# sandialabs/calibr8

Measured on AMD Instinct MI355X. Metric: element Jacobian assemblies/sec, 1M hex8 J2-plasticity fp64, higher is better.
Workload: dtype f64

## Files before the change

### calibr8_amd/csrc/c8_assemble_node.hpp

```cpp
#pragma once

#include "c8_assemble_wave.hpp"

#ifdef C8_STAMPS
#define C8_NSTAMP(i) ex.stamp_node(ga.stamps, node, i)
#else
#define C8_NSTAMP(i)
#endif

namespace c8 {

template <class M, class = void> struct has_closed_form_rows : std::false_type {};
template <class M> struct has_closed_form_rows<M, std::enable_if_t<M::HAS_CLOSED_FORM_ROWS>> : std::true_type {};

template <class E, class ModelD, int MAXDEG, bool MANY> struct NodeShared {
  static constexpr int NR = ModelD::NROW;
  static constexpr int LDR = NR + 4;
  static_assert(LDR % 2 == 0 && (E::NP0 * LDR * 8) % 256 == 128, "record stride: 16-byte aligned, element groups 32 banks apart");
  static constexpr int NREC = 8 * E::NP0 * LDR, NACC = MAXDEG * 16;
  alignas(16) double buf[MANY ? NREC + NACC : (NREC > NACC ? NREC : NACC)];
  alignas(16) double nodal[8][E::NN][4];
  double nshape[8];
  double el[8][2];
  double bsum[4];
  C8_HD double* rec(int s, int pt) { return buf + (s * E::NP0 + pt) * LDR; }
  C8_HD double* img() { return buf + (MANY ? NREC : 0); }
  C8_HD static int img01(int deg) { return 9 * deg; }
  C8_HD static int img10(int deg) { return 12 * deg; }
  C8_HD static int img11(int deg) { return 15 * deg; }
};

C8_HD double const* at_byte(double const* p, int off) { return reinterpret_cast<double const*>(reinterpret_cast<char const*>(p) + off); }

#ifndef C8_TUNE_NODE_HAHEAD
#define C8_TUNE_NODE_HAHEAD 3
#endif

template <int MAXDEG> struct NodeLane {
  static constexpr int N00 = (9 * MAXDEG + 63) / 64, N01 = (3 * MAXDEG + 63) / 64;
  double J[16];
  double a00[N00], a01[N01], a10[N01], a11;
  double bold;
  double rs;
  int e, a, pos;
  bool valid;
};

C8_HD constexpr int hex_code(int n) { return n ^ ((n >> 1) & 1); }
template <class E> C8_HD void hex_pattern(int j, double* v) {
  double c[3], w;
  E::point(0, 7, c, w);
  double const a = 1. + ((j & 1) ? c[0] : -c[0]), b = 1. + ((j & 2) ? c[1] : -c[1]), d = 1. + ((j & 4) ? c[2] : -c[2]);
  v[0] = 0.125 * a * b * d;
  v[1] = 0.125 * b * d;
  v[2] = 0.125 * a * d;
  v[3] = 0.125 * a * b;
}

template <class E> struct HexShape {
  double c[3];
  C8_HD static HexShape of_point(int pt) {
    double w;
    HexShape h;
    E::point(0, pt, h.c, w);
    return h;
  }
  C8_HD double at_node(int n) const {
    double const sx = ((n ^ (n >> 1)) & 1) ? 1. : -1., sy = ((n >> 1) & 1) ? 1. : -1., sz = ((n >> 2) & 1) ? 1. : -1.;
    return 0.125 * (1. + sx * c[0]) * (1. + sy * c[1]) * (1. + sz * c[2]);
  }
  C8_HD static HexShape of_node(int n) {
    HexShape h;
    E::sign(n, h.c[0], h.c[1], h.c[2]);
    return h;
  }
  C8_HD double at_point(int pt) const {
    double xi[3], w;
    E::point(0, pt, xi, w);
    return 0.125 * (1. + c[0] * xi[0]) * (1. + c[1] * xi[1]) * (1. + c[2] * xi[2]);
  }
};

template <class E, template <class> class ModelT, int MAXDEG, bool MANY, bool ADJ = false, class EX>
C8_HD void node_rows_closed(EX& ex, NodeShared<E, ModelT<Dual>, MAXDEG, MANY>& sh, MeshTables const& mt, ModelSettings const& ms,
                            FieldArgs const& fa, GatherArgs const& ga, int node, AdjointArgs const& aa = AdjointArgs{}) {
  using Model = ModelT<Dual>;
  using SH = NodeShared<E, Model, MAXDEG, MANY>;
  using NL_ = NodeLane<MAXDEG>;
  constexpr int NL = Model::NLOC, NR = SH::NR;
  static_assert(E::NN == 8 && E::NP0 == 8 && E::SAME_POINTS, "row-per-node kernel: hex8-like element");
  static_assert(!Mechanics::USES_U && !Model::FINITE_DEF, "row-per-node kernel: small-strain weak form without u terms");
  C8_NSTAMP(6);
  int const nptr = ga.nodeptr[node], deg = ga.nodeptr[node + 1] - nptr;
  int const e0 = ga.nodeelem_ptr[node], e1 = ga.nodeelem_ptr[node + 1];
  size_t const np = (size_t)nptr;
  int const n3 = 3 * deg;
  if (e0 == e1) return;
  C8_NSTAMP(0);
  auto zero_acc = [&](int lane) {
    C8_UNROLL
    for (int it = 0; it < (SH::NACC + 63) / 64; ++it) {
      int const q = lane + 64 * it;
      if (q < 16 * deg) sh.img()[q] = 0.;
    }
    if (lane < 4) sh.bsum[lane] = 0.;
  };
  if (!ADJ || MANY) {
    ex.each([&](int lane) {
      if (!ADJ && lane < 8) {
        double v[4];
        hex_pattern<E>(lane, v);
        sh.nshape[lane] = v[0];
      }
      if (MANY) zero_acc(lane);
    });
    ex.sync();
  }
  for (int c0 = e0; c0 < e1; c0 += 8) {
    int const ne = (e1 - c0 < 8) ? e1 - c0 : 8;
    ex.each([&](int lane) {
      auto& r = ex.lane(lane);
      int const s = lane >> 3, m = lane & 7;
      r.valid = s < ne;
      r.rs = 0.;
      if (!r.valid) return;
      int const packed = ga.nodeelem[c0 + s];
      int const e = packed >> 3, a = packed & 7;
      r.e = e;
      r.a = a;
      r.pos = ga.pos[((size_t)e * E::NN + m) * E::NN + a];
      int const nd = mt.conn[(size_t)e * E::NN + m];
      double* const nv = sh.nodal[s][m];
      nv[0] = fa.u[(size_t)nd * 3 + 0]; nv[1] = fa.u[(size_t)nd * 3 + 1]; nv[2] = fa.u[(size_t)nd * 3 + 2];
      nv[3] = fa.p[nd];
    });
    ex.sync();
    ex.each([&](int lane_) {
      auto& r = ex.lane(lane_);
      int lane = lane_;
      C8_PIN(lane);
      int const s = lane >> 3, pt = lane & 7;
      if (!r.valid) return;
      int const e = r.e, a = r.a;
      double const* const t = mt.shape + (size_t)e * SHAPE_STRIDE;
      size_t const q0 = ((size_t)e * E::NP0 + pt) * NL;
      double G[9], xi_old[NL];
      C8_UNROLL
      for (int c = 0; c < 9; ++c) G[c] = t[SHAPE_JINV + 8 * c + pt];
      if constexpr (!ADJ) {
        C8_UNROLL
        for (int j = 0; j < NL; ++j) xi_old[j] = fa.xi_prev[q0 + j];
      }
      double fh4[4] = {0., 0., 0., 0.}, gx[NL];
      C8_UNROLL
      for (int j = 0; j < NL; ++j) gx[j] = 0.;
      if constexpr (ADJ) {
        double const* const fh = aa.f + ((size_t)e * E::NP0 + pt) * E::NDOF;
        fh4[0] = fh[3 * a + 0]; fh4[1] = fh[3 * a + 1]; fh4[2] = fh[3 * a + 2]; fh4[3] = fh[3 * E::NN + a];
        C8_UNROLL
        for (int j = 0; j < NL; ++j) gx[j] = aa.g[((size_t)e * E::NP0 + pt) * NL + j];
      }
      double q[WQ];
      C8_UNROLL
      for (int c = 0; c < WQ; ++c) q[c] = 0.;
      double g[3];
      {
        double R[12], pN = 0.;
        C8_UNROLL
        for (int c = 0; c < 12; ++c) R[c] = 0.;
        int const mo = hex_code(pt ^ 7) * 32;
        C8_UNROLL
        for (int i = 0; i < E::NN; ++i) {
          double v[4];
          hex_pattern<E>(i, v);
          double const t0 = (i & 1) ? v[1] : -v[1], t1 = (i & 2) ? v[2] : -v[2], t2 = (i & 4) ? v[3] : -v[3];
          double const* const nv = at_byte(sh.nodal[s][0], mo ^ (hex_code(i) * 32));
          double const u0 = nv[0], u1 = nv[1], u2 = nv[2], pm = nv[3];
          R[0] += u0 * t0; R[1] += u0 * t1; R[2] += u0 * t2;
          R[3] += u1 * t0; R[4] += u1 * t1; R[5] += u1 * t2;
          R[6] += u2 * t0; R[7] += u2 * t1; R[8] += u2 * t2;
          pN += pm * v[0];
          R[9] += pm * t0; R[10] += pm * t1; R[11] += pm * t2;
        }
        double const s0 = (pt & 1) ? 1. : -1., s1 = (pt & 2) ? 1. : -1., s2 = (pt & 4) ? 1. : -1.;
        C8_UNROLL
        for (int f = 0; f < 4; ++f) {
          double const r0 = s0 * R[3 * f], r1 = s1 * R[3 * f + 1], r2 = s2 * R[3 * f + 2];
          C8_UNROLL
          for (int d = 0; d < 3; ++d) q[(f < 3 ? 3 * f : 10) + d] = r0 * G[d] + r1 * G[3 + d] + r2 * G[6 + d];
        }
        q[9] = pN;
        double xa[3], wa, da[3];
        E::point(0, pt, xa, wa);
        E::dNdxi(a, xa, da);
        C8_UNROLL
        for (int d = 0; d < 3; ++d) g[d] = da[0] * G[d] + da[1] * G[3 + d] + da[2] * G[6 + d];
      }
      C8_NSTAMP(7);
      if constexpr (ADJ) {
        C8_UNROLL
        for (int j = 0; j < NL; ++j) xi_old[j] = fa.xi_prev[q0 + j];
      }
      int const es = mt.elem_set ? mt.elem_set[e] : 0;
      typename Model::ClosedForm cf;
      Model::closed_form(mt.params + (size_t)es * Model::NPARAMS, q, xi_old, ms.abs_tol, t[SHAPE_H], ms.stab_mult, cf, true);
      if (!ADJ && a == 0) {
        C8_UNROLL
        for (int j = 0; j < NL; ++j) fa.xi[q0 + j] = cf.xi[j];
      }
      C8_NSTAMP(8);
      double const w = t[SHAPE_WDV + pt];
      double Na;
      if constexpr (ADJ) Na = HexShape<E>::of_point(pt).at_node(a);
      else Na = sh.nshape[hex_code(a) ^ pt ^ 7];
      double* const rc = sh.rec(s, pt);
      double el[2];
      Model::template closed_form_row<ADJ>(cf.t, w, g, Na, rc, el);
      if (pt == 0) { sh.el[s][0] = el[0]; sh.el[s][1] = el[1]; }
      if constexpr (!ADJ) {
        C8_UNROLL
        for (int i = 0; i < 3; ++i) rc[NR + i] = w * (cf.F[3 * i] * g[0] + cf.F[3 * i + 1] * g[1] + cf.F[3 * i + 2] * g[2]);
        rc[NR + 3] = w * (cf.F[9] * Na + cf.F[10] * g[0] + cf.F[11] * g[1] + cf.F[12] * g[2]);
      } else {
        double Re[6];
        double dq[10];
        C8_UNROLL
        for (int k = 0; k < 10; ++k) dq[k] = 0.;
        if (aa.qoi.c_load != 0.) {
          double dxi[NL];
          Model::closed_form_load_term(mt.params + (size_t)es * Model::NPARAMS, aa.qoi.c_load * w, aa.qoi.comp,
                                       aa.qoi.S + ((size_t)e * E::NP0 + pt) * 3, dxi, dq);
          C8_UNROLL
          for (int j = 0; j < NL; ++j) gx[j] -= dxi[j];
        }
        Model::closed_form_adjoint(mt.params + (size_t)es * Model::NPARAMS, cf.t, gx, Re);
        double const dJ = aa.qoi.c_avg * w / aa.qoi.ndims * Na;
        rc[NR + 0] = (Re[0] - dq[0]) * g[0] + (Re[1] - dq[1]) * g[1] + (Re[2] - dq[2]) * g[2] - dJ + fh4[0];
        rc[NR + 1] = (Re[1] - dq[3]) * g[0] + (Re[3] - dq[4]) * g[1] + (Re[4] - dq[5]) * g[2] - dJ + fh4[1];
        rc[NR + 2] = (Re[2] - dq[6]) * g[0] + (Re[4] - dq[7]) * g[1] + (Re[5] - dq[8]) * g[2] - dJ + fh4[2];
        rc[NR + 3] = -dq[9] * Na + fh4[3];
      }
    });
    ex.sync();
    C8_NSTAMP(1);
    ex.each([&](int lane_) {
      auto& r = ex.lane(lane_);
      int lane = lane_;
      C8_PIN(lane);
      C8_UNROLL
      for (int j = 0; j < 16; ++j) r.J[j] = 0.;
      if (!r.valid) return;
      int const s = lane >> 3, m = lane & 7;
      double const* const t = mt.shape + (size_t)r.e * SHAPE_STRIDE;
      double const el[2] = {sh.el[s][0], sh.el[s][1]};
      HexShape<E> Nn;
      if constexpr (ADJ) Nn = HexShape<E>::of_node(m);
      constexpr int AH = C8_TUNE_NODE_HAHEAD;
      double hq[AH + 1][3];
      C8_UNROLL
      for (int k = 0; k < AH; ++k) { hq[k][0] = t[k * 24 + m * 2 + 0]; hq[k][1] = t[k * 24 + m * 2 + 1]; hq[k][2] = t[k * 24 + 16 + m]; }
      int off = ((0 - m) & 7) * 8;
      int const cm8 = (hex_code(m) ^ 7) * 8;
      C8_UNROLL
      for (int i = 0; i < E::NP0; ++i) {
        hq[AH][0] = hq[AH][1] = hq[AH][2] = 0.;
        if (i + AH < E::NP0) {
          hq[AH][0] = t[(i + AH) * 24 + m * 2 + 0];
          hq[AH][1] = t[(i + AH) * 24 + m * 2 + 1];
          hq[AH][2] = t[(i + AH) * 24 + 16 + m];
        }
        double const hc[3] = {hq[0][0], hq[0][1], hq[0][2]};
        double Nm;
        if constexpr (ADJ) Nm = Nn.at_point(off >> 3);
        else Nm = *at_byte(sh.nshape, off ^ cm8);
        Model::closed_form_block(at_byte(sh.rec(s, 0), SH::LDR * off), el, hc, Nm, r.J);
        off = (off + 8) & 56;
        C8_UNROLL
        for (int j = 0; j < 16; ++j) C8_PIN(r.J[j]);
        C8_SCHED_FENCE();
        C8_UNROLL
        for (int k = 0; k < AH; ++k) { hq[k][0] = hq[k + 1][0]; hq[k][1] = hq[k + 1][1]; hq[k][2] = hq[k + 1][2]; }
      }
      if (m < 4) {
        double v = 0.;
        C8_UNROLL
        for (int pt = 0; pt < E::NP0; ++pt) v += sh.rec(s, pt)[NR + m];
        r.rs = v;
      }
    });
    C8_NSTAMP(2);
    if (c0 == e0) {
      ex.each([&](int lane_) {
        auto& r = ex.lane(lane_);
        int lane = lane_;
        C8_PIN(lane);
        C8_UNROLL
        for (int it = 0; it < NL_::N00; ++it) {
          int const j = lane + 64 * it;
          r.a00[it] = 0.;
          if (!ga.assign && j < 9 * deg) r.a00[it] = ga.A[0][0][np * 9 + j];
        }
        C8_UNROLL
        for (int it = 0; it < NL_::N01; ++it) {
          int const j = lane + 64 * it;
          r.a01[it] = r.a10[it] = 0.;
          if (!ga.assign && j < n3) { r.a01[it] = ga.A[0][1][np * 3 + j]; r.a10[it] = ga.A[1][0][np * 3 + j]; }
        }
        r.a11 = 0.;
        if (!ga.assign && lane < deg) r.a11 = ga.A[1][1][np + lane];
        r.bold = 0.;
        if (!ga.assign && lane < 4) r.bold = lane < 3 ? ga.b[0][(size_t)node * 3 + lane] : ga.b[1][node];
      });
    }
    if (!MANY) {
      ex.sync();
      ex.each([&](int lane) { zero_acc(lane); });
    }
    ex.sync();
    C8_NSTAMP(3);
    auto add_block = [&](int lane) {
      auto& r = ex.lane(lane);
      double* const c00 = sh.img() + 3 * r.pos;
      double* const c01 = sh.img() + SH::img01(deg) + r.pos;
      double* const c10 = sh.img() + SH::img10(deg) + 3 * r.pos;
      double* const c11 = sh.img() + SH::img11(deg) + r.pos;
      C8_UNROLL
      for (int j = 0; j < 16; ++j) {
        int const i = j >> 2, col = j & 3;
        ex.lds_add(i < 3 ? (col < 3 ? c00 + i * n3 + col : c01 + i * deg) : (col < 3 ? c10 + col : c11), r.J[j]);
      }
      if ((lane & 7) < 4) ex.lds_add(&sh.bsum[lane & 7], r.rs);
    };
#ifndef C8_TUNE_NODE_C_BY_ELEMENT
    ex.each([&](int lane) {
      if ((lane >> 3) >= ne) return;
      add_block(lane);
    });
#else
    for (int s2 = 0; s2 < ne; ++s2) {
      ex.each([&](int lane) {
        if ((lane >> 3) != s2) return;
        add_block(lane);
      });
    }
#endif
    ex.sync();
    C8_NSTAMP(4);
    if (!MANY) break;
  }
  ex.each([&](int lane_) {
    auto& r = ex.lane(lane_);
    int lane = lane_;
    C8_PIN(lane);
    C8_UNROLL
    for (int it = 0; it < NL_::N00; ++it) C8_PIN(r.a00[it]);
    C8_UNROLL
    for (int it = 0; it < NL_::N01; ++it) { C8_PIN(r.a01[it]); C8_PIN(r.a10[it]); }
    C8_PIN(r.a11);
    C8_PIN(r.bold);
    double const* const i00 = sh.img(), * const i01 = i00 + SH::img01(deg), * const i10 = i00 + SH::img10(deg), * const i11 = i00 + SH::img11(deg);
    C8_UNROLL
    for (int it = 0; it < NL_::N00; ++it) {
      int const j = lane + 64 * it;
      if (j < 9 * deg) ga.A[0][0][np * 9 + j] = r.a00[it] + i00[j];
    }
    C8_UNROLL
    for (int it = 0; it < NL_::N01; ++it) {
      int const j = lane + 64 * it;
      if (j < n3) {
        ga.A[0][1][np * 3 + j] = r.a01[it] + i01[j];
        ga.A[1][0][np * 3 + j] = r.a10[it] + i10[j];
      }
    }
    if (lane < deg) ga.A[1][1][np + lane] = r.a11 + i11[lane];
    if (lane < 3) ga.b[0][(size_t)node * 3 + lane] = r.bold + sh.bsum[lane];
    if (lane == 3) ga.b[1][node] = r.bold + sh.bsum[3];
  });
  ex.sync();
  C8_NSTAMP(5);
}

template <class E, template <class> class ModelT>
C8_HD void node_rows_update_g(MeshTables const& mt, AdjointArgs const& aa, size_t qp) {
  using Model = ModelT<Dual>;
  int const e = (int)(qp / E::NP0), pt = (int)(qp % E::NP0);
  int const es = mt.elem_set ? mt.elem_set[e] : 0;
  double const w = mt.shape[(size_t)e * SHAPE_STRIDE + SHAPE_WDV + pt];
  double dxi[Model::NLOC], dq[10];
  Model::closed_form_load_term(mt.params + (size_t)es * Model::NPARAMS, aa.qoi.c_load * w, aa.qoi.comp, aa.qoi.S + qp * 3, dxi, dq);
  C8_UNROLL
  for (int j = 0; j < Model::NLOC; ++j) aa.g[qp * Model::NLOC + j] -= dxi[j];
}

}
```

Before: 273.6 million.

## Prefetch per-point shape data and old state in the gather phase

Loads of the inverse Jacobian, old local state, weight and element size move from the point phase into the earlier gather phase, where they are kept in per-lane registers. The first look-ahead rows for the block phase are also fetched before the closed-form model call, so their latency is hidden behind that compute. The goal is to overlap global-memory latency with the sync and the nodal gathers. In exchange, each lane holds more live state across the barriers, which raises register pressure and may lower occupancy or cause spills.

```diff
diff --git a/calibr8_amd/csrc/c8_assemble_node.hpp b/calibr8_amd/csrc/c8_assemble_node.hpp
--- a/calibr8_amd/csrc/c8_assemble_node.hpp
+++ b/calibr8_amd/csrc/c8_assemble_node.hpp
@@ -36,12 +36,17 @@
 #define C8_TUNE_NODE_HAHEAD 3
 #endif
 
+constexpr int NODE_NXI = 7;
+constexpr int NODE_HQ_EARLY = 2;
+static_assert(NODE_HQ_EARLY <= C8_TUNE_NODE_HAHEAD, "the rows fetched early are rows of phase B's look-ahead");
 template <int MAXDEG> struct NodeLane {
   static constexpr int N00 = (9 * MAXDEG + 63) / 64, N01 = (3 * MAXDEG + 63) / 64;
   double J[16];
   double a00[N00], a01[N01], a10[N01], a11;
   double bold;
   double rs;
+  double G[9], xo[NODE_NXI], w, h;
+  double hq[NODE_HQ_EARLY][3];
   int e, a, pos;
   bool valid;
 };
@@ -88,6 +93,7 @@
   using SH = NodeShared<E, Model, MAXDEG, MANY>;
   using NL_ = NodeLane<MAXDEG>;
   constexpr int NL = Model::NLOC, NR = SH::NR;
+  static_assert(NL <= NODE_NXI, "NodeLane::xo holds a point's local state");
   static_assert(E::NN == 8 && E::NP0 == 8 && E::SAME_POINTS, "row-per-node kernel: hex8-like element");
   static_assert(!Mechanics::USES_U && !Model::FINITE_DEF, "row-per-node kernel: small-strain weak form without u terms");
   C8_NSTAMP(6);
@@ -128,8 +134,20 @@
       int const e = packed >> 3, a = packed & 7;
       r.e = e;
       r.a = a;
+      int const nd = mt.conn[(size_t)e * E::NN + m];
       r.pos = ga.pos[((size_t)e * E::NN + m) * E::NN + a];
-      int const nd = mt.conn[(size_t)e * E::NN + m];
+      {
+        double const* const t = mt.shape + (size_t)e * SHAPE_STRIDE;
+        C8_UNROLL
+        for (int c = 0; c < 9; ++c) r.G[c] = t[SHAPE_JINV + 8 * c + m];
+        if constexpr (!ADJ) {
+          size_t const q0 = ((size_t)e * E::NP0 + m) * NL;
+          C8_UNROLL
+          for (int j = 0; j < NL; ++j) r.xo[j] = fa.xi_prev[q0 + j];
+        }
+        r.w = t[SHAPE_WDV + m];
+        r.h = t[SHAPE_H];
+      }
       double* const nv = sh.nodal[s][m];
       nv[0] = fa.u[(size_t)nd * 3 + 0]; nv[1] = fa.u[(size_t)nd * 3 + 1]; nv[2] = fa.u[(size_t)nd * 3 + 2];
       nv[3] = fa.p[nd];
@@ -146,10 +164,10 @@
       size_t const q0 = ((size_t)e * E::NP0 + pt) * NL;
       double G[9], xi_old[NL];
       C8_UNROLL
-      for (int c = 0; c < 9; ++c) G[c] = t[SHAPE_JINV + 8 * c + pt];
+      for (int c = 0; c < 9; ++c) G[c] = r.G[c];
       if constexpr (!ADJ) {
         C8_UNROLL
-        for (int j = 0; j < NL; ++j) xi_old[j] = fa.xi_prev[q0 + j];
+        for (int j = 0; j < NL; ++j) xi_old[j] = r.xo[j];
       }
       double fh4[4] = {0., 0., 0., 0.}, gx[NL];
       C8_UNROLL
@@ -202,14 +220,16 @@
         for (int j = 0; j < NL; ++j) xi_old[j] = fa.xi_prev[q0 + j];
       }
       int const es = mt.elem_set ? mt.elem_set[e] : 0;
+      C8_UNROLL
+      for (int k = 0; k < NODE_HQ_EARLY; ++k) { r.hq[k][0] = t[k * 24 + pt * 2 + 0]; r.hq[k][1] = t[k * 24 + pt * 2 + 1]; r.hq[k][2] = t[k * 24 + 16 + pt]; }
       typename Model::ClosedForm cf;
-      Model::closed_form(mt.params + (size_t)es * Model::NPARAMS, q, xi_old, ms.abs_tol, t[SHAPE_H], ms.stab_mult, cf, true);
+      Model::closed_form(mt.params + (size_t)es * Model::NPARAMS, q, xi_old, ms.abs_tol, r.h, ms.stab_mult, cf, true);
       if (!ADJ && a == 0) {
         C8_UNROLL
         for (int j = 0; j < NL; ++j) fa.xi[q0 + j] = cf.xi[j];
       }
       C8_NSTAMP(8);
-      double const w = t[SHAPE_WDV + pt];
+      double const w = r.w;
       double Na;
       if constexpr (ADJ) Na = HexShape<E>::of_point(pt).at_node(a);
       else Na = sh.nshape[hex_code(a) ^ pt ^ 7];
@@ -258,7 +278,10 @@
       constexpr int AH = C8_TUNE_NODE_HAHEAD;
       double hq[AH + 1][3];
       C8_UNROLL
-      for (int k = 0; k < AH; ++k) { hq[k][0] = t[k * 24 + m * 2 + 0]; hq[k][1] = t[k * 24 + m * 2 + 1]; hq[k][2] = t[k * 24 + 16 + m]; }
+      for (int k = 0; k < AH; ++k) {
+        if (k < NODE_HQ_EARLY) { hq[k][0] = r.hq[k][0]; hq[k][1] = r.hq[k][1]; hq[k][2] = r.hq[k][2]; }
+        else { hq[k][0] = t[k * 24 + m * 2 + 0]; hq[k][1] = t[k * 24 + m * 2 + 1]; hq[k][2] = t[k * 24 + 16 + m]; }
+      }
       int off = ((0 - m) & 7) * 8;
       int const cm8 = (hex_code(m) ^ 7) * 8;
       C8_UNROLL
```

Result: faster. 278.7 million, median of 6 (+1.8%).
